# rjagerman/glint

Measured on AMD Instinct MI355X. Metric: device-resident push scatter-add GB/s (and % HBM peak) at 1/2/4/8 GPUs, higher is better.
Workload: dtype f64; 1 GPU; north star: dense contiguous-range push scatter-add, 2^30-key Double vector per GPU (BASELINE.json north_star's 1-GPU target configuration); keys_per_gpu=1073741824, key_dtype=i64, parallelism=range-sharded x1, no exchange

## Files before the change

glint_amd/build.py:

```python
from __future__ import annotations

import os
import shutil
import subprocess
import sys
from pathlib import Path

ROOT = Path(__file__).resolve().parent.parent
PKG = ROOT / "glint_amd"
LIB_DIR = PKG / "lib"
LIB = LIB_DIR / "libglint_gpu.so"
ORACLE_DIR = ROOT / "oracle"
ORACLE_LIB = ORACLE_DIR / "build" / "libglint_oracle.so"

CSRC = PKG / "csrc"
HIP_SOURCES = [CSRC / "glint_gpu.hip", CSRC / "glint_sort.hip", CSRC / "glint_route.hip", CSRC / "glint_ordered.hip", CSRC / "glint_bin.hip",
               CSRC / "glint_exchange.hip", CSRC / "glint_rows.hip", CSRC / "glint_sparse.hip",
               CSRC / "glint_rowsum.hip", CSRC / "glint_rowdot.hip", CSRC / "glint_rowaxpy.hip"]
PLAN_HEADERS = [CSRC / "glint_push_plan.h", CSRC / "glint_bin_plan.h"]
HIP_HEADERS = [CSRC / "glint_kernels.h", CSRC / "glint_device.h", CSRC / "glint_host.h", ROOT / "include" / "glint_gpu.h",
               *PLAN_HEADERS]
HIP_DEPS = HIP_SOURCES + HIP_HEADERS
OBJ_DIR = ROOT / "build" / "obj"
ORACLE_SOURCES = [ORACLE_DIR / "glint_oracle.c"]
# ... 33 lines not shown
    for p, obj in procs:
        if p.wait() != 0:
            raise subprocess.CalledProcessError(p.returncode, f"hipcc -c {obj.name}")
        os.replace(str(obj) + ".tmp", obj)
    tmp = LIB.with_suffix(".so.tmp")
    cmd = [_hipcc(), "--offload-arch=gfx950", "-shared", "-fPIC", "-o", str(tmp), *map(str, objs)]
    if verbose:
        print(" ".join(cmd), file=sys.stderr)
    subprocess.run(cmd, check=True, cwd=str(ROOT))
    os.replace(tmp, LIB)
    return LIB


def build_oracle(force: bool = False, verbose: bool = False) -> Path:
    if not force and not _stale(ORACLE_LIB, ORACLE_SOURCES):
        return ORACLE_LIB
    ORACLE_LIB.parent.mkdir(parents=True, exist_ok=True)
    tmp = ORACLE_LIB.with_suffix(".so.tmp")
    cc = shutil.which("gcc") or "cc"
    cmd = [cc, "-O2", "-std=c11", "-fPIC", "-shared", "-fwrapv", "-pthread", "-o", str(tmp),
           *map(str, ORACLE_SOURCES)]
    if verbose:
        print(" ".join(cmd), file=sys.stderr)
    subprocess.run(cmd, check=True, cwd=str(ROOT))
    os.replace(tmp, ORACLE_LIB)
    return ORACLE_LIB


def build_loopback(force: bool = False, verbose: bool = False) -> Path:
    if not force and not _stale(LOOPBACK_BIN, [LOOPBACK_SRC]):
        return LOOPBACK_BIN
    LOOPBACK_BIN.parent.mkdir(parents=True, exist_ok=True)
    tmp = LOOPBACK_BIN.with_suffix(".tmp")
    cc = shutil.which("gcc") or "cc"
    cmd = [cc, "-O2", "-std=c11", "-Wall", "-pthread", "-o", str(tmp), str(LOOPBACK_SRC), "-ldl", "-lm"]
    if verbose:
        print(" ".join(cmd), file=sys.stderr)
    subprocess.run(cmd, check=True, cwd=str(ROOT))
    os.replace(tmp, LOOPBACK_BIN)
    return LOOPBACK_BIN


JNI_SHIM = ROOT / "integration" / "jni" / "glint_jni.c"
JNI_DRIVER_SRC = ROOT / "tests" / "c" / "fake_jvm.c"
JNI_DRIVER = ROOT / "tests" / "c" / "build" / "fake_jvm"


def build_jni_driver(force: bool = False, verbose: bool = False) -> Path:
    deps = [JNI_SHIM, JNI_DRIVER_SRC, ROOT / "tests" / "c" / "jni.h", ROOT / "include" / "glint_gpu.h", LIB]
    if not force and not _stale(JNI_DRIVER, deps):
        return JNI_DRIVER
    JNI_DRIVER.parent.mkdir(parents=True, exist_ok=True)
    tmp = JNI_DRIVER.with_suffix(".tmp")
    cc = shutil.which("gcc") or "cc"
    cmd = [cc, "-O2", "-Wall", "-Werror", "-std=c11", "-I", str(ROOT / "tests" / "c"), "-I", str(ROOT / "include"),
           str(JNI_DRIVER_SRC), str(JNI_SHIM), "-L", str(LIB_DIR), "-lglint_gpu", f"-Wl,-rpath,{LIB_DIR}",
           "-o", str(tmp)]
    if verbose:
        print(" ".join(cmd), file=sys.stderr)
    subprocess.run(cmd, check=True, cwd=str(ROOT))
    os.replace(tmp, JNI_DRIVER)
    return JNI_DRIVER


PLAN_PROBE_SRC = ROOT / "tests" / "c" / "plan_probe.cpp"
PLAN_PROBE = ROOT / "tests" / "c" / "build" / "libplan_probe.so"


def build_plan_probe(force: bool = False, verbose: bool = False) -> Path:
    deps = [PLAN_PROBE_SRC, *PLAN_HEADERS, ROOT / "include" / "glint_gpu.h"]
    if not force and not _stale(PLAN_PROBE, deps):
        return PLAN_PROBE
    PLAN_PROBE.parent.mkdir(parents=True, exist_ok=True)
    tmp = PLAN_PROBE.with_suffix(".so.tmp")
    cxx = shutil.which("g++") or "c++"
    cmd = [cxx, "-O2", "-std=c++17", "-Wall", "-Werror", "-fPIC", "-shared", "-o", str(tmp), str(PLAN_PROBE_SRC)]
    if verbose:
        print(" ".join(cmd), file=sys.stderr)
    subprocess.run(cmd, check=True, cwd=str(ROOT))
    os.replace(tmp, PLAN_PROBE)
    return PLAN_PROBE


def build_all(force: bool = False, verbose: bool = False) -> None:
    build_gpu_lib(force=force, verbose=verbose)
    build_oracle(force=force, verbose=verbose)
    build_loopback(force=force, verbose=verbose)
    build_jni_driver(force=force, verbose=verbose)
    build_plan_probe(force=force, verbose=verbose)


if __name__ == "__main__":
    build_all(force="--force" in sys.argv, verbose=True)
    print(LIB)
    print(ORACLE_LIB)
    print(LOOPBACK_BIN)
```

glint_amd/csrc/glint_bin.hip:

```cpp
#include "glint_device.h"
#include "glint_host.h"
#include "glint_bin_plan.h"

#include <atomic>
#include <cstring>
#include <type_traits>

namespace glint {

constexpr int kAChunk = kATPB * kAPer;
constexpr int kASlots = 2 * kAChunk;
constexpr int kASlotBits = kASlots == 8192 ? 13 : kASlots == 4096 ? 12 : 11;
static_assert((1 << kASlotBits) == kASlots, "dedup table size");
#ifndef GLINT_PART_AHEAD
#define GLINT_PART_AHEAD 2
#endif
constexpr int kPartAhead = GLINT_PART_AHEAD;
#ifndef GLINT_APPLY_TPB
#define GLINT_APPLY_TPB 256
#endif
constexpr int kCTPB = GLINT_APPLY_TPB;
constexpr u32 kEmptySlot = 0xFFFFFFFFu;

__device__ __forceinline__ u32 bucket_of(u32 a, const BinGeom& g) { return a >> (kSlabBits + g.fb); }
// ... 304 lines not shown
        }
      }
    }
  }
  __syncthreads();
  for (int h = tid; h < kHotCount; h += kHotTPB)
    if (cc[h] >= min_count) atomicMax(&best[hot_slot(ck[h])], ((unsigned long long)cc[h] << 32) | ck[h]);
  __syncthreads();
  for (int i = tid; i < kHotSlots; i += kHotTPB) hot_tags[i] = best[i] ? (u32)best[i] : kEmptySlot;
}

template <typename A> __device__ __forceinline__ A hot_zero() { return A(0); }
template <> __device__ __forceinline__ double hot_zero<double>() { return -0.0; }
template <typename A> __device__ __forceinline__ bool hot_untouched(A x) { return x == A(0); }
template <> __device__ __forceinline__ bool hot_untouched<double>(double x) {
  return __double_as_longlong(x) == (long long)0x8000000000000000ull;
}
__device__ __forceinline__ void hot_flush(double* p, double x) { gadd(p, x); }
__device__ __forceinline__ void hot_flush(float* p, double x) { gadd(p, (float)x); }
__device__ __forceinline__ void hot_flush(long long* p, long long x) { gadd(p, x); }
__device__ __forceinline__ void hot_flush(int* p, int x) { gadd(p, x); }

template <typename A, int P>
__device__ __forceinline__ u32 part_emit(const u32 (&ad)[P], const A (&va)[P], u32 valid, const BinGeom& g,
                                         u32* dcnt, u32* gcnt, u32* st_a, A* st_v, const BufOut& ctb, u32 ctcol,
                                         u32 ctstride, u32* __restrict__ out_a, A* __restrict__ out_v, PhaseClock& ph,
                                         int pb) {
  const int tid = threadIdx.x;
  u32 rank[P];
#pragma unroll
  for (int j = 0; j < P; ++j)
    if (valid & (1u << j)) rank[j] = atomicAdd(&dcnt[bucket_of(ad[j], g)], 1u);
  __syncthreads();
  ph.mark(pb);
  const u32 total = block_scan<kATPB, 1>(
      g.nb, [&](u32 d) { return dcnt[d]; },
      [&](u32 d, u32 excl) {
        gcnt[d] = dcnt[d];
        dcnt[d] = excl;
      });
  ph.mark(pb + 1);
  static_assert(kMaxDigit <= kATPB, "one chunk-table entry per thread, for up to kMaxDigit buckets");
  bput(ctb, ((u32)tid * ctstride + ctcol) * 4u, (u32)tid < g.nb, dcnt[tid] | (gcnt[tid] << 16));
#pragma unroll
  for (int j = 0; j < P; ++j) {
    if (valid & (1u << j)) {
      const u32 p = dcnt[bucket_of(ad[j], g)] + rank[j];
      st_a[p] = ad[j];
      st_v[p] = va[j];
    }
  }
  __syncthreads();
  ph.mark(pb + 2);
  const RecOut<u32> oa{buf_out(out_a, total * 4u)};
  const RecOut<A> ov{buf_out(out_v, total * (u32)sizeof(A))};
#pragma unroll
  for (int j = 0; j < P; ++j) {
    if ((u32)(j * kATPB) >= total) break;
    const u32 p = tid + j * kATPB;
    const bool on = p < total;
    oa.put(p, on, st_a[p]);
    ov.put(p, on, st_v[p]);
  }
  __syncthreads();
  ph.mark(pb + 3);
  for (u32 d = tid; d < g.nb; d += kATPB) dcnt[d] = 0;
  __syncthreads();
  ph.mark(pb + 4);
  return total;
}

__device__ __forceinline__ void part_next_header(const BinGeom& g, BinCtl* next_bc, u32* __restrict__ next_T,
                                                 LaunchCtl* next_ctl) {
  const int tid = threadIdx.x;
  for (u32 b = tid; b < kMaxDigit; b += kATPB) {
    next_T[b] = 0;
    next_T[kMaxDigit + b] = 0;
  }
  if (tid < (int)(sizeof(BinCtl) / 4)) reinterpret_cast<u32*>(next_bc)[tid] = 0;
  if (next_ctl && tid == 0) {
    next_ctl->brk_enc = 0u;
    next_ctl->nonaffine = 0u;
    next_ctl->cancel = 0u;
    next_ctl->bad = 0ull;
  }
}

__device__ __forceinline__ u32 bucket_items(u32 t, u32 item) { return max(1u, (t + item - 1) / item); }

constexpr int kWideHashBits = 20;
constexpr int kWideRunsPerWg = 8;
constexpr int kWideSampleWgs = 256;

template <bool MAT>
__global__ __launch_bounds__(256) void bin_hot_sample_kernel(const i64* __restrict__ keys, const int32_t* __restrict__ cols,
                                                             i64 n, PartDesc part, const LaunchCtl* lctl, u32 ntiles,
                                                             int from_break, u32* __restrict__ gkey,
                                                             u32* __restrict__ gcnt) {
  constexpr int kLocal = 2048;
  __shared__ u32 lk[kLocal], lc[kLocal];
  const int tid = threadIdx.x;
  for (int i = tid; i < kLocal; i += 256) {
    lk[i] = kEmptySlot;
    lc[i] = 0;
  }
  __syncthreads();
  const i64 r0 = tail_start(lctl, ntiles, from_break, n);
  const i64 m = n - r0;
  const i64 runs = (i64)kWideSampleWgs * kWideRunsPerWg;
  if (m > 0) {
    const i64 stride = m >= runs * kHotRun ? m / runs : kHotRun;
    constexpr int kPer = kWideRunsPerWg * kHotRun / 256;
#pragma unroll
    for (int j = 0; j < kPer; ++j) {
      const int s = j * 256 + tid;
      const i64 run = (i64)blockIdx.x * kWideRunsPerWg + s / kHotRun;
      const i64 i = r0 + run * stride + s % kHotRun;
      if (i >= n) continue;
      i64 a64;
      if (!rec_addr<MAT>(part, keys[i], MAT ? cols[i] : 0, a64)) continue;
      const u32 a = (u32)a64;
      u32 h = hot_mix(a * 0x9E3779B1u) & (kLocal - 1);
      for (int probe = 0; probe < 64; ++probe) {
        const u32 prev = atomicCAS(&lk[h], kEmptySlot, a);
        if (prev == kEmptySlot || prev == a) {
          atomicAdd(&lc[h], 1u);
          break;
        }
        h = (h + 1) & (kLocal - 1);
      }
    }
  }
  __syncthreads();
  constexpr u32 kMask = (1u << kWideHashBits) - 1u;
  for (int i = tid; i < kLocal; i += 256) {
    const u32 a = lk[i];
    if (a == kEmptySlot) continue;
    u32 h = hot_mix(a) & kMask;
    for (int probe = 0; probe < 64; ++probe) {
      const u32 prev = atomicCAS(&gkey[h], kEmptySlot, a);
      if (prev == kEmptySlot || prev == a) {
        atomicAdd(&gcnt[h], lc[i]);
        break;
      }
      h = (h + 1) & kMask;
    }
  }
}

__global__ __launch_bounds__(256) void bin_hot_select_kernel(u32* __restrict__ gkey, u32* __restrict__ gcnt,
                                                             u32 min_count, unsigned long long* __restrict__ best) {
  const u32 i = blockIdx.x * 256u + threadIdx.x;
  const u32 a = gkey[i], c = gcnt[i];
  gkey[i] = kEmptySlot;
  gcnt[i] = 0;
  if (a != kEmptySlot && c >= min_count) atomicMax(&best[wide_slot(a)], ((unsigned long long)c << 32) | a);
}

constexpr int kRedSlots = 64, kRedTPB = 1024, kRedGroups = kRedTPB / kRedSlots;
template <typename V>
__device__ __forceinline__ void hot_reduce_block(u32 blk, const unsigned long long* __restrict__ best, u32 G,
                                                 const typename LdsAcc<V>::T* __restrict__ partial,
                                                 V* __restrict__ data, const LaunchCtl* gated) {
  typedef typename LdsAcc<V>::T A;
  if (gated && gated->cancel) return;
  __shared__ A gs[kRedGroups][kRedSlots];
// ... 1350 lines not shown
```

glint_amd/csrc/glint_gpu.hip:

```cpp
#include "glint_kernels.h"
#include "../../include/glint_gpu.h"
#include "glint_device.h"

#include <mutex>
#include <vector>
#include <utility>
#include <new>
#include <chrono>
#include <cstring>
#include <sched.h>
#include <time.h>
#include <cstdio>
#include <algorithm>
#include <cstdlib>

namespace glint {

template <bool MAT> struct AddrT { typedef int32_t T; };
template <> struct AddrT<true> { typedef i64 T; };

template <bool MAT, int KIND = -1>
__device__ __forceinline__ bool rec_addr_t(const PartDesc& p, i64 key, int32_t col, typename AddrT<MAT>::T& addr) {
  i64 ad;
  const bool ok = rec_addr<MAT, KIND>(p, key, col, ad);
  addr = (typename AddrT<MAT>::T)ad;
  return ok;
}

template <bool MAT, bool FULL, int KIND>
__device__ __forceinline__ bool check_tile(const i64* __restrict__ keys, const int32_t* __restrict__ cols, i64 n,
                                           const PartDesc& part, LaunchCtl* ctl, i64* __restrict__ desc,
                                           u32 ntiles, u32 t, int lane, bool validate, bool read_all) {
  typedef typename AddrT<MAT>::T A;
  const i64 pbase = (i64)t * (kTile / 2);
  K2 k[kPPT];
  C2 c[kPPT];
#pragma unroll
  for (int j = 0; j < kPPT; ++j) {
    const i64 p = pbase + lane + (i64)j * 64;
    const i64 r = 2 * p;
    if (FULL || r + 1 < n) {
      k[j] = __builtin_nontemporal_load(reinterpret_cast<const K2*>(keys) + p);
      if (MAT) c[j] = __builtin_nontemporal_load(reinterpret_cast<const C2*>(cols) + p);
    } else {
      k[j] = K2{r < n ? keys[r] : 0, 0};
      if (MAT) c[j] = C2{r < n ? cols[r] : 0, 0};
    }
  }
  const i64 r_first = 2 * pbase;
  const i64 kb = r_first > 0 ? keys[r_first - 1] : 0;
  const int32_t cb = (MAT && r_first > 0) ? cols[r_first - 1] : 0;
  const u32 brk = __builtin_amdgcn_readfirstlane(ld_relaxed(&ctl->brk_enc));
  const bool after = brk != 0u && ntiles - brk < t;
  if (!read_all && after) return false;
  A before = 0;
  if (r_first > 0) rec_addr_t<MAT, KIND>(part, kb, cb, before);
  bool mono = true, affine = true;
  A a_first = 0;
  A last = before;
#pragma unroll
  for (int j = 0; j < kPPT; ++j) {
    const i64 r = 2 * (pbase + lane + (i64)j * 64);
    const bool h0 = FULL || r < n, h1 = FULL || r + 1 < n;
    A a0, a1;
    const bool o0 = rec_addr_t<MAT, KIND>(part, k[j].x, MAT ? c[j].x : 0, a0);
    const bool o1 = rec_addr_t<MAT, KIND>(part, k[j].y, MAT ? c[j].y : 0, a1);
    if (j == 0) a_first = __shfl(a0, 0);
    if (h1) mono = mono && (a1 > a0);
    A prev = __shfl_up(a1, 1);
    if (lane == 0) prev = last;
    if (h0 && r > 0) mono = mono && (a0 > prev);
    last = __shfl(a1, 63);
    const A off = (A)(r - r_first);
    affine = affine && (!h0 || (o0 && a0 == a_first + off)) && (!h1 || (o1 && a1 == a_first + off + 1));
    if (validate) {
      const bool b0 = h0 && (!o0 || !key_in_part<KIND>(part, k[j].x));
      const bool b1 = h1 && (!o1 || !key_in_part<KIND>(part, k[j].y));
      if (b0 || b1) atomicMax(&ctl->bad, ~(u64)(b0 ? r : r + 1));
    }
  }
  const bool any_bad = __any(!mono);
  const bool all_affine = __all(affine);
  if (lane == 0 && !after) {
    if (any_bad) {
      if (ld_relaxed(&ctl->brk_enc) < ntiles - t) atomicMax(&ctl->brk_enc, ntiles - t);
    } else {
      desc[t] = all_affine ? (i64)a_first : kNotAffine;
      const bool linked = all_affine && (r_first == 0 || (i64)a_first == (i64)before + 1);
      if (!linked && ld_relaxed(&ctl->nonaffine) == 0u) atomicOr(&ctl->nonaffine, 1u);
    }
  }
  return true;
}

template <bool MAT, int KIND>
__global__ __launch_bounds__(kTPB) void push_check_kernel(const i64* __restrict__ keys,
                                                          const int32_t* __restrict__ cols, i64 n,
                                                          PartDesc part, LaunchCtl* ctl, LaunchCtl* next,
                                                          i64* __restrict__ desc, u32 ntiles, u32 t_begin,
                                                          u32 t_end, int validate) {
  const int lane = threadIdx.x & 63;
  if (t_begin == 0 && blockIdx.x == 0 && threadIdx.x == 0) {
    next->brk_enc = 0u;
    next->nonaffine = 0u;
    next->cancel = 0u;
    next->bad = 0ull;
  }
  if (ctl->cancel) return;
  const u32 w0 = blockIdx.x * (kTPB / 64) + (threadIdx.x >> 6);
  const u32 nw = gridDim.x * (kTPB / 64);
  for (u32 t = t_begin + w0; t < t_end; t += nw) {
    const bool full = 2 * ((i64)t * (kTile / 2)) + kTile <= n;
    const bool go = full ? check_tile<MAT, true, KIND>(keys, cols, n, part, ctl, desc, ntiles, t, lane, validate != 0,
                                                       validate == 1)
                         : check_tile<MAT, false, KIND>(keys, cols, n, part, ctl, desc, ntiles, t, lane, validate != 0,
                                                        validate == 1);
    if (!go) return;
  }
}

template <typename V, bool MAT, bool FULL>
__device__ __forceinline__ void apply_affine(const PushArgs<V>& a, i64 pbase, i64 base, int lane) {
  typedef typename Vec2<V>::T V2;
  const i64 n = a.n;
  const i64 r_first = 2 * pbase;
  V2 v[kPPT], d[kPPT];
  if ((base & 1) == 0) {
    V2* dp = reinterpret_cast<V2*>(a.data + base);
#pragma unroll
    for (int j = 0; j < kPPT; ++j) {
      const i64 q = lane + (i64)j * 64;
      if (FULL || 2 * (pbase + q) + 1 < n) {
        v[j] = __builtin_nontemporal_load(reinterpret_cast<const V2*>(a.vals) + pbase + q);
        d[j] = dp[q];
      }
    }
#pragma unroll
    for (int j = 0; j < kPPT; ++j) {
      const i64 q = lane + (i64)j * 64;
      const i64 r = 2 * (pbase + q);
      if (FULL || r + 1 < n) dp[q] = as2<V>(vadd((V)d[j].x, (V)v[j].x), vadd((V)d[j].y, (V)v[j].y));
      else if (r < n) a.data[base + (r - r_first)] = vadd(a.data[base + (r - r_first)], a.vals[r]);
    }
  } else {
#pragma unroll
    for (int j = 0; j < kPPT; ++j) {
      const i64 p = pbase + lane + (i64)j * 64;
      const i64 r = 2 * p;
      const i64 e = base + (r - r_first);
      if (FULL || r + 1 < n) {
        v[j] = __builtin_nontemporal_load(reinterpret_cast<const V2*>(a.vals) + p);
        d[j] = as2<V>(a.data[e], a.data[e + 1]);
      } else {
        v[j] = as2<V>(r < n ? a.vals[r] : V(0), V(0));
        d[j] = as2<V>(r < n ? a.data[e] : V(0), V(0));
      }
    }
#pragma unroll
    for (int j = 0; j < kPPT; ++j) {
      const i64 r = 2 * (pbase + lane + (i64)j * 64);
      const i64 e = base + (r - r_first);
      if (FULL || r < n) a.data[e] = vadd((V)d[j].x, (V)v[j].x);
      if (FULL || r + 1 < n) a.data[e + 1] = vadd((V)d[j].y, (V)v[j].y);
    }
  }
}

template <typename V, bool MAT, bool FULL>
__device__ __forceinline__ void apply_general(const PushArgs<V>& a, i64 pbase, int lane) {
  typedef typename Vec2<V>::T V2;
  typedef typename AddrT<MAT>::T A;
  const i64 n = a.n;
  K2 k[kPPT];
  C2 c[kPPT];
  V2 v[kPPT];
#pragma unroll
  for (int j = 0; j < kPPT; ++j) {
    const i64 p = pbase + lane + (i64)j * 64;
    const i64 r = 2 * p;
    if (FULL || r + 1 < n) {
      k[j] = __builtin_nontemporal_load(reinterpret_cast<const K2*>(a.keys) + p);
      if (MAT) c[j] = __builtin_nontemporal_load(reinterpret_cast<const C2*>(a.cols) + p);
      v[j] = __builtin_nontemporal_load(reinterpret_cast<const V2*>(a.vals) + p);
    } else {
      k[j] = K2{r < n ? a.keys[r] : 0, 0};
      if (MAT) c[j] = C2{r < n ? a.cols[r] : 0, 0};
      v[j] = as2<V>(r < n ? a.vals[r] : V(0), V(0));
    }
  }
#pragma unroll
  for (int j = 0; j < kPPT; ++j) {
    const i64 r = 2 * (pbase + lane + (i64)j * 64);
    A a0, a1;
    const bool h0 = FULL || r < n, h1 = FULL || r + 1 < n;
    const bool o0 = rec_addr_t<MAT>(a.part, k[j].x, MAT ? c[j].x : 0, a0) && h0;
    const bool o1 = rec_addr_t<MAT>(a.part, k[j].y, MAT ? c[j].y : 0, a1) && h1;
    if (h0 && !o0) record_error(a.err, r);
    if (h1 && !o1) record_error(a.err, r + 1);
    if (o0 && o1 && a1 == a0 + 1 && (a0 & 1) == 0) {
      V2* dp = reinterpret_cast<V2*>(a.data + a0);
      const V2 d = *dp;
      *dp = as2<V>(vadd((V)d.x, (V)v[j].x), vadd((V)d.y, (V)v[j].y));
    } else {
      if (o0) a.data[a0] = vadd(a.data[a0], (V)v[j].x);
      if (o1) a.data[a1] = vadd(a.data[a1], (V)v[j].y);
    }
  }
}

constexpr int kSweepU = 2;
template <typename V, bool EVEN>
__device__ __forceinline__ void apply_sweep(const PushArgs<V>& a, i64 delta, i64 p_begin, i64 p_end, bool last) {
  typedef typename Vec2<V>::T V2;
  if (blockIdx.x >= a.sweep_blocks) return;
  const i64 npairs = p_end;
  const i64 stride = (i64)a.sweep_blocks * kTPB;
  const V2* vp = reinterpret_cast<const V2*>(a.vals);
  i64 p = p_begin + (i64)blockIdx.x * kTPB + threadIdx.x;
  if (EVEN) {
    V2* dp = reinterpret_cast<V2*>(a.data + delta);
    for (; p + (kSweepU - 1) * stride < npairs; p += kSweepU * stride) {
      V2 v[kSweepU], d[kSweepU];
#pragma unroll
      for (int j = 0; j < kSweepU; ++j) {
        v[j] = __builtin_nontemporal_load(vp + p + j * stride);
        d[j] = __builtin_nontemporal_load(dp + p + j * stride);
      }
#pragma unroll
      for (int j = 0; j < kSweepU; ++j)
        __builtin_nontemporal_store(as2<V>(vadd((V)d[j].x, (V)v[j].x), vadd((V)d[j].y, (V)v[j].y)), dp + p + j * stride);
    }
    for (; p < npairs; p += stride) {
      const V2 v = __builtin_nontemporal_load(vp + p);
      const V2 d = __builtin_nontemporal_load(dp + p);
      __builtin_nontemporal_store(as2<V>(vadd((V)d.x, (V)v.x), vadd((V)d.y, (V)v.y)), dp + p);
    }
  } else {
    for (; p < npairs; p += stride) {
      const V2 v = __builtin_nontemporal_load(vp + p);
      const i64 e = 2 * p + delta;
      const V d0 = a.data[e], d1 = a.data[e + 1];
      a.data[e] = vadd(d0, (V)v.x);
      a.data[e + 1] = vadd(d1, (V)v.y);
    }
  }
  if ((a.n & 1) && last && blockIdx.x == 0 && threadIdx.x == 0) {
    const i64 e = a.n - 1 + delta;
    a.data[e] = vadd(a.data[e], a.vals[a.n - 1]);
  }
}

template <typename V, bool MAT>
__global__ __launch_bounds__(kTPB) void push_apply_kernel(PushArgs<V> a, const i64* __restrict__ desc, u32 t_begin,
                                                          u32 t_end) {
  if (a.ctl->cancel) return;
  const u32 brk = a.ctl->brk_enc;
  if (t_begin == 0 && blockIdx.x == 0 && threadIdx.x == 0 && a.hint) {
    __hip_atomic_store(a.hint, brk == 0u ? 0ull : (u64)(a.n - (i64)(a.ntiles - brk) * kTile), __ATOMIC_RELAXED,
                       __HIP_MEMORY_SCOPE_SYSTEM);
    __hip_atomic_store(a.hint + 3, brk == 0u ? (u64)a.n : (u64)(a.ntiles - brk) * kTile, __ATOMIC_RELAXED,
                       __HIP_MEMORY_SCOPE_SYSTEM);
  }
  if (brk == 0u && a.ctl->nonaffine == 0u) {
    const i64 delta = desc[0];
    const i64 p0 = (i64)t_begin * (kTile / 2), p1 = min((i64)t_end * (kTile / 2), a.n >> 1);
    const bool last = t_end >= a.ntiles;
    if ((delta & 1) == 0) apply_sweep<V, true>(a, delta, p0, p1, last);
    else apply_sweep<V, false>(a, delta, p0, p1, last);
    return;
  }
  const u32 tiles = min(t_end, brk == 0u ? a.ntiles : a.ntiles - brk);
  const int lane = threadIdx.x & 63;
  const u32 w0 = blockIdx.x * (kTPB / 64) + (threadIdx.x >> 6);
  const u32 nw = gridDim.x * (kTPB / 64);
  i64 dbatch = kNotAffine;
  for (u32 t = t_begin + w0, it = 0; t < tiles; t += nw, ++it) {
    if ((it & 63) == 0) {
      const i64 tt = (i64)t + (i64)lane * nw;
      dbatch = tt < (i64)tiles ? desc[tt] : kNotAffine;
    }
    const i64 pbase = (i64)t * (kTile / 2);
    const i64 base = __shfl(dbatch, (int)(it & 63));
    const bool full = 2 * pbase + kTile <= a.n;
    if (base != kNotAffine) {
      if (full) apply_affine<V, MAT, true>(a, pbase, base, lane);
      else apply_affine<V, MAT, false>(a, pbase, base, lane);
    } else {
      if (full) apply_general<V, MAT, true>(a, pbase, lane);
      else apply_general<V, MAT, false>(a, pbase, lane);
    }
  }
}


constexpr u64 kEmpty = ~0ull;

template <typename V, bool MAT>
__global__ __launch_bounds__(kTPB) void push_scatter_kernel(PushArgs<V> a, int force_all) {
  i64 r0 = 0;
  if (force_all == 2 && blockIdx.x == 0 && threadIdx.x == 0 && a.hint) {
    __hip_atomic_store(a.hint, (u64)a.n, __ATOMIC_RELAXED, __HIP_MEMORY_SCOPE_SYSTEM);
    __hip_atomic_store(a.hint + 3, 0ull, __ATOMIC_RELAXED, __HIP_MEMORY_SCOPE_SYSTEM);
  }
  if (!force_all) {
    const u32 brk = a.ctl->brk_enc;
    if (brk == 0u) return;
    r0 = (i64)(a.ntiles - brk) * kTile;
  }
  if (r0 >= a.n) return;
  const i64 rem = a.n - r0;
  const i64 nchunks = (rem + kScatterChunk - 1) / kScatterChunk;
  if ((i64)blockIdx.x >= nchunks) return;

  typedef typename LdsAcc<V>::T A;
  __shared__ u64 hk[kHashSlots];
  __shared__ A hv[kHashSlots];
  const int tid = threadIdx.x;
  for (int s = tid; s < kHashSlots; s += kTPB) { hk[s] = kEmpty; hv[s] = A(0); }
  __syncthreads();

  for (i64 ch = blockIdx.x; ch < nchunks; ch += gridDim.x) {
    const i64 cbase = r0 + ch * kScatterChunk;
#pragma unroll 2
    for (int q = tid; q < kScatterChunk; q += kTPB) {
      const i64 i = cbase + q;
      if (i >= a.n) break;
      const i64 key = a.keys[i];
      const int32_t col = MAT ? a.cols[i] : 0;
      const V val = a.vals[i];
      i64 addr;
      if (!rec_addr<MAT>(a.part, key, col, addr)) { record_error(a.err, i); continue; }
      const u64 ua = (u64)addr;
      u32 h = (u32)((ua * 0x9E3779B97F4A7C15ull) >> (64 - 12));
      for (;;) {
        const u64 cur = __hip_atomic_load(&hk[h], __ATOMIC_RELAXED, __HIP_MEMORY_SCOPE_WORKGROUP);
        if (cur == ua) break;
        if (cur == kEmpty) {
          const u64 prev = atomicCAS(&hk[h], kEmpty, ua);
          if (prev == kEmpty || prev == ua) break;
        }
        h = (h + 1) & (kHashSlots - 1);
      }
      lds_add(&hv[h], (A)val);
    }
    __syncthreads();
    for (int s = tid; s < kHashSlots; s += kTPB) {
      const u64 key = hk[s];
      if (key != kEmpty) {
        gadd(a.data + key, (V)hv[s]);
        hk[s] = kEmpty;
        hv[s] = A(0);
      }
    }
    __syncthreads();
  }
}

constexpr int kMaxSetShards = 64;
template <typename V>
struct ShardSet {
  int n;
  i64 start[kMaxSetShards];
  i64 end[kMaxSetShards];
  V* data[kMaxSetShards];
};

__device__ __forceinline__ int set_find(const i64* st, const i64* en, int n, i64 key) {
  int lo = 0, hi = n;
  while (lo < hi) {
    const int mid = (lo + hi) >> 1;
    if (st[mid] <= key) lo = mid + 1;
    else hi = mid;
  }
// ... 311 lines not shown
                  kTPB, st, a.keys, a.cols, a.n, a.part, a.ctl, next, desc, a.ntiles, 0u, a.ntiles, vmode));
  return GLINT_OK;
}

template <typename V, bool MAT>
int launch_push(glint_shard* s, const i64* keys, const int32_t* cols, const void* vals, i64 n, int flags,
                hipStream_t st) {
  if (n <= 0) return GLINT_OK;
  if (!keys || !vals || (MAT && !cols)) return GLINT_EINVAL;
  PushArgs<V> a;
  a.keys = keys;
  a.cols = cols;
  a.vals = (const V*)vals;
  a.n = n;
  a.data = (V*)s->data;
  a.part = s->part;
  a.err = err_of(s);
  a.elems = s->elems;
  a.hint = s->d_hint;
  a.sig = s->sig;
  a.sweep_blocks = 0;
  const i64 ntiles = (n + kTile - 1) / kTile;
  if (ntiles >= (i64)0xFFFFFFF0ll) return GLINT_EINVAL;
  a.ntiles = (u32)ntiles;

  PushQuery q;
  q.n = n;
  q.flags = flags;
  q.fp = s->dtype == GLINT_F32 || s->dtype == GLINT_F64;
  q.vec_ok = aligned(keys, 16) && aligned(vals, 2 * sizeof(V)) && (!MAT || aligned(cols, 8));
  q.gated = s->gate != nullptr;
  q.ring = a.sig.done != nullptr;
  q.elems = s->elems;
  q.binnable = push_binnable(s, n);
  q.hint_tail = s->hint_tail;
  q.hint_head = s->hint_head;
  q.whole_probe = s->whole_probe;
  q.binned_mode = binned_mode();
  q.bin_density = bin_density();
  q.whole_on = whole_on();
  const PushRoute r = push_route(q);
  if (r.kind == PushKind::Invalid) return GLINT_EINVAL;
  if (r.kind == PushKind::Ordered) return push_ordered<V, MAT>(s, a, st);

  const size_t ctl_need = 256 + (size_t)ntiles * sizeof(i64);
  const void* ctl_old = s->d_ctl;
  int rc = grow(&s->d_ctl, &s->ctl_bytes, ctl_need);
  if (rc) return rc;
  if (s->d_ctl != ctl_old) {
    HIPCHK(hipMemsetAsync(s->d_ctl, 0, 2 * sizeof(LaunchCtl), st));
    s->ctl_par = 0;
  }
  LaunchCtl* const slots = (LaunchCtl*)s->d_ctl;
  a.ctl = slots + s->ctl_par;
  LaunchCtl* const next = slots + (s->ctl_par ^ 1);
  i64* desc = (i64*)((char*)s->d_ctl + 256);
  if (r.probe_consumed) ++s->whole_probe;

  switch (r.kind) {
    case PushKind::BinnedAll: return push_binned<V, MAT>(s, a, false, st);
    case PushKind::WholeBin: {
      const BinHook hook = [&](void* bc, u32* T, u32 nb) -> int {
        return launch_validate_gate_binned(a.ctl, s->gate, bc, T, nb, st);
      };
      rc = push_binned<V, MAT>(s, a, false, st, r.validate ? &hook : nullptr, next);
      if (rc == GLINT_OK) s->ctl_par ^= 1;
      return rc;
    }
    case PushKind::DetAll: return push_det_tail<V, MAT>(s, a, false, st);
    case PushKind::ScatterAll: return launch_scatter<V, MAT>(s, a, r.scatter_mode, st);
    default: break;
  }
  if (r.gate_kernel) {
    push_gate_kernel<<<1, 64, 0, st>>>(s->gate, a.ctl);
    HIPCHK(hipGetLastError());
  }
  rc = launch_check<V, MAT>(s, a, next, desc, r.validate ? (r.fuse ? 2 : 1) : 0, st);
  if (rc) return rc;
  if (r.validate && !r.fuse) {
    push_validate_gate_kernel<<<1, 64, 0, st>>>(a.ctl, s->gate);
    HIPCHK(hipGetLastError());
  }
  s->ctl_par ^= 1;
  const u64 win = std::min<u64>(kSweepWindowTiles, a.ntiles);
  auto apply_head = [&]() -> int {
    const i64 bpc = blocks_per_cu<push_apply_kernel<V, MAT>>(2);
    for (u64 t0 = 0; t0 < a.ntiles; t0 += win) {
      const u32 t1 = (u32)std::min<u64>(a.ntiles, t0 + win);
      const unsigned ga = grid_for(t1 - t0, kTPB / 64, (i64)s->cus * bpc);
      a.sweep_blocks = std::min<u32>(ga, (u32)((i64)s->cus * kSweepBlocksPerCu));
      HIPCHK(launch_k(s, GLINT_K_PUSH_APPLY, push_apply_kernel<V, MAT>, ga, kTPB, st, a, (const i64*)desc, (u32)t0, t1));
    }
    return GLINT_OK;
  };
  if (r.fuse) {
    const BinHook hook = [&](void* bc, u32* T, u32 nb) -> int {
      const int rc2 = launch_validate_gate_binned(a.ctl, s->gate, bc, T, nb, st);
      return rc2 ? rc2 : apply_head();
    };
    return push_binned<V, MAT>(s, a, true, st, &hook);
  }
  rc = apply_head();
  if (rc) return rc;
  switch (r.tail) {
    case PushTail::Det: return push_det_tail<V, MAT>(s, a, true, st);
    case PushTail::Binned: return push_binned<V, MAT>(s, a, true, st);
    default: return launch_scatter<V, MAT>(s, a, 0, st);
  }
}

template <typename V>
int launch_vec_pull(glint_shard* s, const i64* keys, void* out, i64 n, hipStream_t st) {
  if (n <= 0) return GLINT_OK;
  if (!keys || !out) return GLINT_EINVAL;
  const MsgSig sig = s->sig;
  if (sig.done && n <= kRingPullMax) {
    HIPCHK(launch_k(s, GLINT_K_VEC_PULL, ring_pull_kernel<V, false>, 1u, kRingPullTPB, st, keys, (const int32_t*)nullptr,
                    n, (const V*)s->data, s->part, (V*)out, err_of(s), sig, s->pull_tab, s->pull_nm));
    return GLINT_OK;
  }
  const bool pairs = aligned(keys, 16) && aligned(out, 2 * sizeof(V));
  if (pairs) {
    const i64 npairs = (n + 1) / 2;
    const i64 win = sig.done ? npairs : std::min<i64>(npairs, (i64)kSweepWindowTiles * (kTile / 2));
    for (i64 p0 = 0; p0 < npairs; p0 += win) {
      const i64 p1 = std::min<i64>(npairs, p0 + win);
      const unsigned g = sig.done ? 1u : grid_for(p1 - p0, kTPB, (i64)s->cus * kPullBlocksPerCu);
      HIPCHK(launch_k(s, GLINT_K_VEC_PULL, vec_pull_kernel<V, true>, g, kTPB, st, keys, n, (const V*)s->data, s->part,
                      (V*)out, err_of(s), sig, p0, p1));
    }
  } else {
    const unsigned g = sig.done ? 1u : grid_for(n, kTPB, (i64)s->cus * 8);
    HIPCHK(launch_k(s, GLINT_K_VEC_PULL, vec_pull_kernel<V, false>, g, kTPB, st, keys, n, (const V*)s->data, s->part,
                    (V*)out, err_of(s), sig, (i64)0, (i64)0));
  }
  return GLINT_OK;
}

template <typename V>
int launch_mat_pull(glint_shard* s, const i64* rows, const int32_t* cols, void* out, i64 n, hipStream_t st) {
  if (n <= 0) return GLINT_OK;
  if (!rows || !cols || !out) return GLINT_EINVAL;
  const MsgSig sig = s->sig;
  if (sig.done && n <= kRingPullMax) {
    HIPCHK(launch_k(s, GLINT_K_MAT_PULL, ring_pull_kernel<V, true>, 1u, kRingPullTPB, st, rows, cols, n,
                    (const V*)s->data, s->part, (V*)out, err_of(s), sig, s->pull_tab, s->pull_nm));
    return GLINT_OK;
  }
  const unsigned g = sig.done ? 1u : grid_for(n, kTPB, (i64)s->cus * 8);
  HIPCHK(launch_k(s, GLINT_K_MAT_PULL, mat_pull_kernel<V>, g, kTPB, st, rows, cols, n, (const V*)s->data, s->part,
                  (V*)out, err_of(s), sig));
  return GLINT_OK;
}

template <typename V>
int launch_mat_pull_rows(glint_shard* s, const i64* rows, void* out, i64 n, hipStream_t st) {
  if (n <= 0) return GLINT_OK;
  if (!rows || !out) return GLINT_EINVAL;
  const MsgSig sig = s->sig;
  const bool v16 = ((i64)s->part.cols * (i64)sizeof(V)) % 16 == 0 && aligned(out, 16);
  const unsigned g = sig.done ? 1u : grid_for(n, kTPB / 64, (i64)s->cus * 8);
  HIPCHK(launch_k(s, GLINT_K_MAT_PULL_ROWS, v16 ? mat_pull_rows_kernel<V, true> : mat_pull_rows_kernel<V, false>, g,
                  kTPB, st, rows, n, (const V*)s->data, s->part, (V*)out, err_of(s), sig));
  return GLINT_OK;
}

#define GLINT_DISPATCH(dt, FN, ...)                            \
  switch (dt) {                                                \
    case GLINT_F64: return FN<double>(__VA_ARGS__);            \
    case GLINT_F32: return FN<float>(__VA_ARGS__);             \
    case GLINT_I64: return FN<long long>(__VA_ARGS__);         \
    case GLINT_I32: return FN<int>(__VA_ARGS__);               \
    default: return GLINT_EINVAL;                              \
  }

// ... 1789 lines not shown
```

glint_amd/csrc/glint_kernels.h:

```cpp
#pragma once
#include <hip/hip_runtime.h>
#include <stdint.h>

#include "glint_push_plan.h"

namespace glint {

constexpr int kTPB = 256;
constexpr i64 kNotAffine = (i64)0x8000000000000000ll;
constexpr int kHashSlots = 4096;
constexpr int kScatterChunk = 2048;

struct LaunchCtl {
  u32 brk_enc;
  u32 nonaffine;
  u32 cancel;
  u32 pad_;
  u64 bad;
};

struct ErrState {
  u64 min_bad_enc;
  u64 count;
};

struct MsgSig {
  u64* done;
  u64 ticket;
  ErrState* herr;
};

struct PullDst {
  unsigned int off, n;
  unsigned long long dst;
};
constexpr int kPullDirectMax = 256;

struct PartDesc {
  int32_t kind;
  int32_t size;
  int64_t start;
  int32_t cidx;
  int32_t cparts;
  int32_t cols;
  int32_t pad_;
  int64_t pitch;
};

template <int KIND = -1>
__device__ __forceinline__ int32_t g2l(const PartDesc& p, i64 key) {
  if (KIND == 0 || (KIND < 0 && p.kind == 0)) return (int32_t)(key - p.start);
  return (int32_t)((key - (i64)p.cidx) / (i64)p.cparts);
}

template <typename V, int VPL, bool WIDE>
__device__ __forceinline__ void slice_load(V (&x)[VPL], const V* __restrict__ row, i64 c, i64 cols) {
  typedef __attribute__((ext_vector_type(4))) unsigned int U4;
  if (WIDE) {
    U4 q = {0u, 0u, 0u, 0u};
    if (c < cols) q = *reinterpret_cast<const U4*>(row + c);
    __builtin_memcpy(x, &q, 16);
  } else {
#pragma unroll
    for (int k = 0; k < VPL; ++k) {
      const i64 cc = c + (i64)k * 64;
      x[k] = cc < cols ? row[cc] : V(0);
    }
  }
}

template <typename V, int VPL, bool WIDE>
__device__ __forceinline__ void slice_store(const V (&x)[VPL], V* row, i64 c, i64 cols) {
  typedef __attribute__((ext_vector_type(4))) unsigned int U4;
  if (WIDE) {
    U4 q;
    __builtin_memcpy(&q, x, 16);
    if (c < cols) *reinterpret_cast<U4*>(row + c) = q;
  } else {
#pragma unroll
    for (int k = 0; k < VPL; ++k) {
      const i64 cc = c + (i64)k * 64;
      if (cc < cols) row[cc] = x[k];
    }
  }
}

template <typename V>
struct PushArgs {
  const i64* keys;
  const int32_t* cols;
  const V* vals;
  i64 n;
  V* data;
  i64 elems;
  PartDesc part;
  LaunchCtl* ctl;
  u32 ntiles;
  ErrState* err;
  u32 sweep_blocks;
  u64* hint;
// ... 5 lines not shown
```

glint_amd/csrc/glint_push_plan.h:

```cpp
#pragma once
#include "../../include/glint_gpu.h"

#include <stddef.h>
#include <stdint.h>

namespace glint {

typedef long long i64;
typedef unsigned long long u64;
typedef unsigned int u32;

constexpr int kPPT = 8;
constexpr int kTile = 64 * kPPT * 2;
constexpr i64 kOrderedMax = (i64)1 << 17;
constexpr int kPushHostSequential = 1 << 16;
constexpr i64 kSmallPushMax = 4096;
constexpr i64 kBinMin = (i64)1 << 20;

inline size_t pad256(size_t b) { return (b + 255) & ~(size_t)255; }

struct PushQuery {
  i64 n = 0;
  int flags = 0;
  bool fp = false;
  bool vec_ok = false;
  bool gated = false;
  bool ring = false;
  i64 elems = 0;
  bool binnable = false;
  u64 hint_tail = 0;
  u64 hint_head = 0;
  u32 whole_probe = 0;
  int binned_mode = -1;
  i64 bin_density = 512;
  bool whole_on = true;
};

enum class PushKind {
  Invalid,
  Ordered,
  BinnedAll,
  WholeBin,
  ScatterAll,
  DetAll,
  Checked
};
enum class PushTail { Scatter, Det, Binned };

struct PushRoute {
  PushKind kind = PushKind::Invalid;
  PushTail tail = PushTail::Scatter;
  bool validate = false;
  bool fuse = false;
  bool gate_kernel = false;
  int scatter_mode = 0;
  bool probe_consumed = false;
};

inline PushRoute push_route(const PushQuery& q) {
  PushRoute r;
  const bool det = (q.flags & GLINT_PUSH_DETERMINISTIC) && q.fp;
  const bool unordered = (q.flags & GLINT_PUSH_UNORDERED) != 0;
  const bool seq = det || (q.fp && (q.flags & kPushHostSequential) && !unordered);
  if (q.gated && (det || !q.vec_ok)) return r;
  if (q.ring || (seq && q.n <= kOrderedMax && q.elems < ((i64)1 << 32))) {
    r.kind = PushKind::Ordered;
    return r;
  }
  const i64 last_tail = (i64)q.hint_tail;
  const i64 slabs = (q.elems + 4095) / 4096;
  const bool binned =
      !det && q.vec_ok && q.binnable && q.binned_mode != 0 &&
      (unordered || (q.n >= kBinMin && (q.binned_mode == 1 ||
                                        (last_tail >= kBinMin && last_tail >= q.bin_density * slabs))));
  if (binned && unordered && !q.gated) {
    r.kind = PushKind::BinnedAll;
    return r;
  }
  r.validate = q.gated && (q.flags & GLINT_PUSH_VALIDATE) != 0;
  const bool from_zero = q.hint_tail > 0 && q.hint_head == 0;
  if (binned && (!q.gated || r.validate) && from_zero && q.whole_on) {
    r.kind = PushKind::WholeBin;
    return r;
  }
  const bool small = !det && !q.gated && q.n <= kSmallPushMax;
  r.probe_consumed = !binned && !det && !q.gated && q.vec_ok && !small && from_zero;
  const bool whole_scatter = r.probe_consumed && (q.whole_probe & 7u) != 7u && q.whole_on;
  if (!q.vec_ok || small || whole_scatter) {
    r.kind = det ? PushKind::DetAll : PushKind::ScatterAll;
    r.scatter_mode = whole_scatter ? 2 : 1;
    return r;
  }
  r.kind = PushKind::Checked;
  r.gate_kernel = q.gated && !r.validate;
  r.fuse = r.validate && binned && !det;
  r.tail = det ? PushTail::Det : binned ? PushTail::Binned : PushTail::Scatter;
  return r;
}

struct BinFrontState {
  double chunk_ratio = 1.0;
  double hot_frac = 0.0;
  u32 pushes = 0;
  int last_front = 0;
  u32 hot_age = 0;
};

}
```

Before: 6240 GB/s.

## Replace windowed multi-launch apply with single launch using atomic ticket work distribution

The push apply stage used to launch one kernel per window of tiles, each with a static grid-stride split. It now makes a single launch in which blocks take fixed-size row-chunk tickets from an atomic counter stored in LaunchCtl, and the counter is reset in the next-launch header. This removes the repeated launch overhead and the tail imbalance between blocks, but adds one atomic per ticket, a __syncthreads per ticket, and a different access pattern that could affect DRAM locality.

```diff
diff --git a/glint_amd/build.py b/glint_amd/build.py
--- a/glint_amd/build.py
+++ b/glint_amd/build.py
@@ -139,12 +139,32 @@
     return PLAN_PROBE
 
 
+SWEEP_PROBE_SRC = ROOT / "tests" / "c" / "sweep_probe.cpp"
+SWEEP_PROBE = ROOT / "tests" / "c" / "build" / "libsweep_probe.so"
+
+
+def build_sweep_probe(force: bool = False, verbose: bool = False) -> Path:
+    deps = [SWEEP_PROBE_SRC, *PLAN_HEADERS, ROOT / "include" / "glint_gpu.h"]
+    if not force and not _stale(SWEEP_PROBE, deps):
+        return SWEEP_PROBE
+    SWEEP_PROBE.parent.mkdir(parents=True, exist_ok=True)
+    tmp = SWEEP_PROBE.with_suffix(".so.tmp")
+    cxx = shutil.which("g++") or "c++"
+    cmd = [cxx, "-O2", "-std=c++17", "-Wall", "-Werror", "-fPIC", "-shared", "-o", str(tmp), str(SWEEP_PROBE_SRC)]
+    if verbose:
+        print(" ".join(cmd), file=sys.stderr)
+    subprocess.run(cmd, check=True, cwd=str(ROOT))
+    os.replace(tmp, SWEEP_PROBE)
+    return SWEEP_PROBE
+
+
 def build_all(force: bool = False, verbose: bool = False) -> None:
     build_gpu_lib(force=force, verbose=verbose)
     build_oracle(force=force, verbose=verbose)
     build_loopback(force=force, verbose=verbose)
     build_jni_driver(force=force, verbose=verbose)
     build_plan_probe(force=force, verbose=verbose)
+    build_sweep_probe(force=force, verbose=verbose)
 
 
 if __name__ == "__main__":
diff --git a/glint_amd/csrc/glint_bin.hip b/glint_amd/csrc/glint_bin.hip
--- a/glint_amd/csrc/glint_bin.hip
+++ b/glint_amd/csrc/glint_bin.hip
@@ -410,6 +410,7 @@
     next_ctl->brk_enc = 0u;
     next_ctl->nonaffine = 0u;
     next_ctl->cancel = 0u;
+    next_ctl->ticket = 0u;
     next_ctl->bad = 0ull;
   }
 }
diff --git a/glint_amd/csrc/glint_gpu.hip b/glint_amd/csrc/glint_gpu.hip
--- a/glint_amd/csrc/glint_gpu.hip
+++ b/glint_amd/csrc/glint_gpu.hip
@@ -104,6 +104,7 @@
     next->brk_enc = 0u;
     next->nonaffine = 0u;
     next->cancel = 0u;
+    next->ticket = 0u;
     next->bad = 0ull;
   }
   if (ctl->cancel) return;
@@ -209,53 +210,67 @@
 }
 
 constexpr int kSweepU = 2;
+static_assert(kSweepRowPairs == kTPB && kSweepTicketRows % kSweepU == 0, "a ticket row is one pair per thread");
 template <typename V, bool EVEN>
-__device__ __forceinline__ void apply_sweep(const PushArgs<V>& a, i64 delta, i64 p_begin, i64 p_end, bool last) {
+__device__ __forceinline__ void apply_sweep(const PushArgs<V>& a, i64 delta, u32* next_ticket) {
   typedef typename Vec2<V>::T V2;
   if (blockIdx.x >= a.sweep_blocks) return;
-  const i64 npairs = p_end;
-  const i64 stride = (i64)a.sweep_blocks * kTPB;
+  const u32 S = a.sweep_blocks;
+  const i64 npairs = a.n >> 1;
+  const u32 ntickets = (u32)sweep_ticket_count(a.n, S);
+  const bool counted = ntickets > S;
   const V2* vp = reinterpret_cast<const V2*>(a.vals);
-  i64 p = p_begin + (i64)blockIdx.x * kTPB + threadIdx.x;
-  if (EVEN) {
-    V2* dp = reinterpret_cast<V2*>(a.data + delta);
-    for (; p + (kSweepU - 1) * stride < npairs; p += kSweepU * stride) {
-      V2 v[kSweepU], d[kSweepU];
+  V2* dp = reinterpret_cast<V2*>(a.data + (EVEN ? delta : 0));
+  u32 t = blockIdx.x;
+  for (int it = 0; t < ntickets; ++it) {
+    u32 nx = ntickets;
+    if (counted && threadIdx.x == 0) nx = S + atomicAdd(&a.ctl->ticket, 1u);
+    const SweepTicket k = sweep_ticket(t, S);
+    i64 p = k.first + threadIdx.x;
+    int r = 0;
+    if (EVEN && k.first + (kSweepTicketRows - 1) * k.stride + kSweepRowPairs <= npairs) {
+      for (; r < kSweepTicketRows; r += kSweepU, p += kSweepU * k.stride) {
+        V2 v[kSweepU], d[kSweepU];
 #pragma unroll
-      for (int j = 0; j < kSweepU; ++j) {
-        v[j] = __builtin_nontemporal_load(vp + p + j * stride);
-        d[j] = __builtin_nontemporal_load(dp + p + j * stride);
+        for (int j = 0; j < kSweepU; ++j) {
+          v[j] = __builtin_nontemporal_load(vp + p + j * k.stride);
+          d[j] = __builtin_nontemporal_load(dp + p + j * k.stride);
+        }
+#pragma unroll
+        for (int j = 0; j < kSweepU; ++j)
+          __builtin_nontemporal_store(as2<V>(vadd((V)d[j].x, (V)v[j].x), vadd((V)d[j].y, (V)v[j].y)), dp + p + j * k.stride);
       }
-#pragma unroll
-      for (int j = 0; j < kSweepU; ++j)
-        __builtin_nontemporal_store(as2<V>(vadd((V)d[j].x, (V)v[j].x), vadd((V)d[j].y, (V)v[j].y)), dp + p + j * stride);
-    }
-    for (; p < npairs; p += stride) {
+    }
+    for (; r < kSweepTicketRows; ++r, p += k.stride) {
+      if (p >= npairs) break;
       const V2 v = __builtin_nontemporal_load(vp + p);
-      const V2 d = __builtin_nontemporal_load(dp + p);
-      __builtin_nontemporal_store(as2<V>(vadd((V)d.x, (V)v.x), vadd((V)d.y, (V)v.y)), dp + p);
-    }
-  } else {
-    for (; p < npairs; p += stride) {
-      const V2 v = __builtin_nontemporal_load(vp + p);
-      const i64 e = 2 * p + delta;
-      const V d0 = a.data[e], d1 = a.data[e + 1];
-      a.data[e] = vadd(d0, (V)v.x);
-      a.data[e + 1] = vadd(d1, (V)v.y);
-    }
-  }
-  if ((a.n & 1) && last && blockIdx.x == 0 && threadIdx.x == 0) {
+      if (EVEN) {
+        const V2 d = __builtin_nontemporal_load(dp + p);
+        __builtin_nontemporal_store(as2<V>(vadd((V)d.x, (V)v.x), vadd((V)d.y, (V)v.y)), dp + p);
+      } else {
+        const i64 e = 2 * p + delta;
+        const V d0 = a.data[e], d1 = a.data[e + 1];
+        a.data[e] = vadd(d0, (V)v.x);
+        a.data[e + 1] = vadd(d1, (V)v.y);
+      }
+    }
+    if (!counted) break;
+    if (threadIdx.x == 0) next_ticket[it & 1] = nx;
+    __syncthreads();
+    t = next_ticket[it & 1];
+  }
+  if ((a.n & 1) && blockIdx.x == 0 && threadIdx.x == 0) {
     const i64 e = a.n - 1 + delta;
     a.data[e] = vadd(a.data[e], a.vals[a.n - 1]);
   }
 }
 
 template <typename V, bool MAT>
-__global__ __launch_bounds__(kTPB) void push_apply_kernel(PushArgs<V> a, const i64* __restrict__ desc, u32 t_begin,
-                                                          u32 t_end) {
+__global__ __launch_bounds__(kTPB) void push_apply_kernel(PushArgs<V> a, const i64* __restrict__ desc) {
+  __shared__ u32 next_ticket[2];
   if (a.ctl->cancel) return;
   const u32 brk = a.ctl->brk_enc;
-  if (t_begin == 0 && blockIdx.x == 0 && threadIdx.x == 0 && a.hint) {
+  if (blockIdx.x == 0 && threadIdx.x == 0 && a.hint) {
     __hip_atomic_store(a.hint, brk == 0u ? 0ull : (u64)(a.n - (i64)(a.ntiles - brk) * kTile), __ATOMIC_RELAXED,
                        __HIP_MEMORY_SCOPE_SYSTEM);
     __hip_atomic_store(a.hint + 3, brk == 0u ? (u64)a.n : (u64)(a.ntiles - brk) * kTile, __ATOMIC_RELAXED,
@@ -263,32 +278,42 @@
   }
   if (brk == 0u && a.ctl->nonaffine == 0u) {
     const i64 delta = desc[0];
-    const i64 p0 = (i64)t_begin * (kTile / 2), p1 = min((i64)t_end * (kTile / 2), a.n >> 1);
-    const bool last = t_end >= a.ntiles;
-    if ((delta & 1) == 0) apply_sweep<V, true>(a, delta, p0, p1, last);
-    else apply_sweep<V, false>(a, delta, p0, p1, last);
+    if ((delta & 1) == 0) apply_sweep<V, true>(a, delta, next_ticket);
+    else apply_sweep<V, false>(a, delta, next_ticket);
     return;
   }
-  const u32 tiles = min(t_end, brk == 0u ? a.ntiles : a.ntiles - brk);
+  static_assert(kTileRowTiles == kTPB / 64 && kTileTicketRows <= 64, "a ticket row is one tile per wave");
+  const i64 tiles = brk == 0u ? a.ntiles : a.ntiles - brk;
   const int lane = threadIdx.x & 63;
-  const u32 w0 = blockIdx.x * (kTPB / 64) + (threadIdx.x >> 6);
-  const u32 nw = gridDim.x * (kTPB / 64);
-  i64 dbatch = kNotAffine;
-  for (u32 t = t_begin + w0, it = 0; t < tiles; t += nw, ++it) {
-    if ((it & 63) == 0) {
-      const i64 tt = (i64)t + (i64)lane * nw;
-      dbatch = tt < (i64)tiles ? desc[tt] : kNotAffine;
-    }
-    const i64 pbase = (i64)t * (kTile / 2);
-    const i64 base = __shfl(dbatch, (int)(it & 63));
-    const bool full = 2 * pbase + kTile <= a.n;
-    if (base != kNotAffine) {
-      if (full) apply_affine<V, MAT, true>(a, pbase, base, lane);
-      else apply_affine<V, MAT, false>(a, pbase, base, lane);
-    } else {
-      if (full) apply_general<V, MAT, true>(a, pbase, lane);
-      else apply_general<V, MAT, false>(a, pbase, lane);
-    }
+  const u32 G = gridDim.x;
+  const u32 ntickets = (u32)tile_ticket_count(tiles, G);
+  const bool counted = ntickets > G;
+  u32 tk = blockIdx.x;
+  for (int it = 0; tk < ntickets; ++it) {
+    u32 nx = ntickets;
+    if (counted && threadIdx.x == 0) nx = G + atomicAdd(&a.ctl->ticket, 1u);
+    const SweepTicket k = tile_ticket(tk, G);
+    const i64 t0 = k.first + (threadIdx.x >> 6);
+    const i64 tt = t0 + (i64)lane * k.stride;
+    const i64 dbatch = lane < kTileTicketRows && tt < tiles ? desc[tt] : kNotAffine;
+    for (int r = 0; r < kTileTicketRows; ++r) {
+      const i64 t = t0 + (i64)r * k.stride;
+      if (t >= tiles) break;
+      const i64 pbase = t * (kTile / 2);
+      const i64 base = __shfl(dbatch, r);
+      const bool full = 2 * pbase + kTile <= a.n;
+      if (base != kNotAffine) {
+        if (full) apply_affine<V, MAT, true>(a, pbase, base, lane);
+        else apply_affine<V, MAT, false>(a, pbase, base, lane);
+      } else {
+        if (full) apply_general<V, MAT, true>(a, pbase, lane);
+        else apply_general<V, MAT, false>(a, pbase, lane);
+      }
+    }
+    if (!counted) break;
+    if (threadIdx.x == 0) next_ticket[it & 1] = nx;
+    __syncthreads();
+    tk = next_ticket[it & 1];
   }
 }
 
@@ -766,15 +791,10 @@
     HIPCHK(hipGetLastError());
   }
   s->ctl_par ^= 1;
-  const u64 win = std::min<u64>(kSweepWindowTiles, a.ntiles);
   auto apply_head = [&]() -> int {
-    const i64 bpc = blocks_per_cu<push_apply_kernel<V, MAT>>(2);
-    for (u64 t0 = 0; t0 < a.ntiles; t0 += win) {
-      const u32 t1 = (u32)std::min<u64>(a.ntiles, t0 + win);
-      const unsigned ga = grid_for(t1 - t0, kTPB / 64, (i64)s->cus * bpc);
-      a.sweep_blocks = std::min<u32>(ga, (u32)((i64)s->cus * kSweepBlocksPerCu));
-      HIPCHK(launch_k(s, GLINT_K_PUSH_APPLY, push_apply_kernel<V, MAT>, ga, kTPB, st, a, (const i64*)desc, (u32)t0, t1));
-    }
+    const unsigned ga = grid_for(a.ntiles, kTPB / 64, (i64)s->cus * blocks_per_cu<push_apply_kernel<V, MAT>>(2));
+    a.sweep_blocks = std::min<u32>(ga, (u32)((i64)s->cus * kSweepBlocksPerCu));
+    HIPCHK(launch_k(s, GLINT_K_PUSH_APPLY, push_apply_kernel<V, MAT>, ga, kTPB, st, a, (const i64*)desc));
     return GLINT_OK;
   };
   if (r.fuse) {
diff --git a/glint_amd/csrc/glint_kernels.h b/glint_amd/csrc/glint_kernels.h
--- a/glint_amd/csrc/glint_kernels.h
+++ b/glint_amd/csrc/glint_kernels.h
@@ -15,7 +15,7 @@
   u32 brk_enc;
   u32 nonaffine;
   u32 cancel;
-  u32 pad_;
+  u32 ticket;
   u64 bad;
 };
 
diff --git a/glint_amd/csrc/glint_push_plan.h b/glint_amd/csrc/glint_push_plan.h
--- a/glint_amd/csrc/glint_push_plan.h
+++ b/glint_amd/csrc/glint_push_plan.h
@@ -98,6 +98,40 @@
   return r;
 }
 
+#if defined(__HIPCC__)
+#define GLINT_HD __host__ __device__
+#else
+#define GLINT_HD
+#endif
+constexpr int kSweepRowPairs = 256;
+constexpr int kSweepTicketRows = 16;
+constexpr i64 kSweepTicketRecords = 2ll * kSweepTicketRows * kSweepRowPairs;
+
+struct SweepTicket {
+  i64 first;
+  i64 stride;
+};
+
+GLINT_HD inline u64 ticket_count(i64 units, i64 row, int rows, u32 S) {
+  const i64 sw = row * rows * (i64)S;
+  const i64 rem_rows = (units % sw + row - 1) / row;
+  return (u64)(units / sw) * S + (u64)(rem_rows < (i64)S ? rem_rows : (i64)S);
+}
+GLINT_HD inline SweepTicket ticket_at(u64 t, i64 row, int rows, u32 S) {
+  SweepTicket k;
+  k.stride = (i64)S * row;
+  k.first = (i64)(t / S) * rows * k.stride + (i64)(t % S) * row;
+  return k;
+}
+
+GLINT_HD inline u64 sweep_ticket_count(i64 n, u32 S) { return ticket_count(n >> 1, kSweepRowPairs, kSweepTicketRows, S); }
+GLINT_HD inline SweepTicket sweep_ticket(u64 t, u32 S) { return ticket_at(t, kSweepRowPairs, kSweepTicketRows, S); }
+
+constexpr int kTileRowTiles = 4;
+constexpr int kTileTicketRows = 8;
+GLINT_HD inline u64 tile_ticket_count(i64 tiles, u32 G) { return ticket_count(tiles, kTileRowTiles, kTileTicketRows, G); }
+GLINT_HD inline SweepTicket tile_ticket(u64 t, u32 G) { return ticket_at(t, kTileRowTiles, kTileTicketRows, G); }
+
 struct BinFrontState {
   double chunk_ratio = 1.0;
   double hot_frac = 0.0;
```

Measured after the change: 6450 GB/s, median of 6. +3.4%, better.
